# enoche/MMRec

Measured on NVIDIA H100. Metric: graph-prop edges/sec (+ full-catalog scored-items/sec in extra) @ d=64, higher is better.
Workload: dtype f32

## Files before the change

### mmrec_b200/csrc/project_tc.cu

```cuda
#include "tc_common.cuh"

namespace mmrec {

using namespace tc;

constexpr int PJ_M = 128;
constexpr int PJ_KC = 32;
constexpr int PJ_LBO_A = 2064;
constexpr int PJ_A_BYTES = (PJ_KC / 4) * PJ_LBO_A;
constexpr int PJ_CONV = 256;
constexpr int PJ_THREADS = PJ_CONV + 32;
template <int N> constexpr int pj_depth() { return N == 64 ? 3 : (N == 128 ? 2 : 1); }

struct ProjParams {
    const float* table; int64_t F; const int64_t* idx; int64_t n_out;
    const float *Whi, *Wlo;
    int N, n_chunks, chunks_per_split, n_splits, stages, vec_ok, n_tiles;
    float* partial;
    int64_t rows_padded;
};

struct PjSmem {
    uint32_t a0, b0, bars, total, stage_bytes, b_bytes;
};
__host__ __device__ inline PjSmem pj_smem(int N, int stages) {
    PjSmem L;
    L.b_bytes = (uint32_t)N * PJ_KC * 4;
    L.stage_bytes = 2 * PJ_A_BYTES + 2 * L.b_bytes;
    L.a0 = 0;
    L.b0 = 2 * PJ_A_BYTES;
    L.bars = stages * L.stage_bytes;
    L.total = L.bars + 32 * 8;
    return L;
}

template <int N, bool FAST>
__global__ void __launch_bounds__(PJ_THREADS, 1) project_tc_kernel(const ProjParams p) {
    constexpr int PJ_DEPTH = pj_depth<N>();
    extern __shared__ __align__(1024) uint8_t smem[];
    const PjSmem L = pj_smem(N, p.stages);
    const uint32_t sbase = smem_u32(smem);
    const uint32_t bar = sbase + L.bars;
    const int warp = threadIdx.x >> 5, lane = threadIdx.x & 31;
    if (threadIdx.x == 0) {
        for (int s = 0; s < 8; ++s) { mbar_init(bar + s * 8, PJ_CONV); mbar_init(bar + (8 + s) * 8, 1); mbar_init(bar + (16 + s) * 8, PJ_CONV / 32); }
        mbar_fence_init();
    }
    __syncthreads();

    const int tile = blockIdx.x / p.n_splits, sp = blockIdx.x % p.n_splits;
    const int c0 = sp * p.chunks_per_split;
    const int c1 = min(p.n_chunks, c0 + p.chunks_per_split);
    const int n_my = c1 - c0;
    const int rot = n_my > 0 ? ((int)(((int64_t)tile * n_my) / p.n_tiles) / PJ_DEPTH * PJ_DEPTH) % n_my : 0;

    if (warp == PJ_CONV / 32) {
        if (lane == 0) {
            int s = 0;
            uint32_t par = 1;
            for (int c = 0; c < n_my; ++c) {
                mbar_wait(bar + (16 + s) * 8, par);
                mbar_expect_tx(bar + (8 + s) * 8, 2 * L.b_bytes);
                const int64_t off = (int64_t)(c0 + (c + rot) % n_my) * (L.b_bytes / 4);
                bulk_g2s(sbase + s * L.stage_bytes + L.b0, p.Whi + off, L.b_bytes, bar + (8 + s) * 8);
                bulk_g2s(sbase + s * L.stage_bytes + L.b0 + L.b_bytes, p.Wlo + off, L.b_bytes, bar + (8 + s) * 8);
                if (++s == p.stages) { s = 0; par ^= 1; }
            }
        }
        return;
    }
    const int t = threadIdx.x;
    const int g = t >> 7;
    const int kb = t & 7;
    const float* rowp[4];
#pragma unroll
    for (int i = 0; i < 4; ++i) {
        const int64_t r = (int64_t)tile * PJ_M + (t >> 3) + 32 * i;
        rowp[i] = r < p.n_out ? p.table + (p.idx ? p.idx[r] : r) * p.F : nullptr;
    }
    int ld_c = rot;
    const float* kp[4];
#pragma unroll
    for (int i = 0; i < 4; ++i) kp[i] = rowp[i] ? rowp[i] + (int64_t)c0 * PJ_KC + kb * 4 : nullptr;
    auto load_chunk = [&](int c, float4 (&x)[4]) {
        if (FAST) {
            const bool on = c < n_my;
#pragma unroll
            for (int i = 0; i < 4; ++i)
                x[i] = (on && kp[i]) ? __ldg(reinterpret_cast<const float4*>(kp[i] + ld_c * PJ_KC)) : make_float4(0.f, 0.f, 0.f, 0.f);
            if (on && ++ld_c == n_my) ld_c = 0;
            return;
        }
        const int64_t k = (int64_t)(c0 + (c + rot) % n_my) * PJ_KC + kb * 4;
#pragma unroll
        for (int i = 0; i < 4; ++i) {
            float4 v = make_float4(0.f, 0.f, 0.f, 0.f);
            if (rowp[i] && c < n_my) {
                if (p.vec_ok && k + 3 < p.F) v = __ldg(reinterpret_cast<const float4*>(rowp[i] + k));
                else {
                    if (k + 0 < p.F) v.x = __ldg(rowp[i] + k + 0);
                    if (k + 1 < p.F) v.y = __ldg(rowp[i] + k + 1);
                    if (k + 2 < p.F) v.z = __ldg(rowp[i] + k + 2);
                    if (k + 3 < p.F) v.w = __ldg(rowp[i] + k + 3);
                }
            }
            x[i] = v;
        }
    };
    const uint32_t LBO_B = (uint32_t)(N / 8) * 128;
    const uint64_t a_hi0 = smem_desc(sbase + L.a0 + g * 1024, PJ_LBO_A, 128), a_lo0 = smem_desc(sbase + L.a0 + PJ_A_BYTES + g * 1024, PJ_LBO_A, 128);
    const uint64_t b_hi0 = smem_desc(sbase + L.b0, LBO_B, 128), b_lo0 = smem_desc(sbase + L.b0 + L.b_bytes, LBO_B, 128);
    const uint64_t ka = (2 * PJ_LBO_A) >> 4, kbs = (2 * LBO_B) >> 4;
    float acc[N / 2];
#pragma unroll
    for (int i = 0; i < N / 2; ++i) acc[i] = 0.f;
    uint32_t first = 0;
    int prev = 0;
    float4 ringA[PJ_DEPTH][4], ringB[PJ_DEPTH][4];
    int s = 0;
    uint32_t par = 1;
    int done = 0;
    auto fill = [&](int cbase, float4 (&ring)[PJ_DEPTH][4]) {
#pragma unroll
        for (int q = 0; q < PJ_DEPTH; ++q) load_chunk(cbase + q, ring[q]);
    };
    auto drain = [&](int cbase, float4 (&ring)[PJ_DEPTH][4]) {
#pragma unroll
        for (int q = 0; q < PJ_DEPTH; ++q) {
            if (cbase + q < n_my) {
                mbar_wait(bar + (16 + s) * 8, par);
                uint8_t* st = smem + s * L.stage_bytes;
#pragma unroll
                for (int i = 0; i < 4; ++i) {
                    const int r = (t >> 3) + 32 * i;
                    const uint32_t off = kb * PJ_LBO_A + (r >> 3) * 128 + (r & 7) * 16;
                    float4 h, l;
                    split_tf32_trunc(ring[q][i].x, h.x, l.x); split_tf32_trunc(ring[q][i].y, h.y, l.y);
                    split_tf32_trunc(ring[q][i].z, h.z, l.z); split_tf32_trunc(ring[q][i].w, h.w, l.w);
                    *reinterpret_cast<float4*>(st + L.a0 + off) = h;
                    *reinterpret_cast<float4*>(st + L.a0 + PJ_A_BYTES + off) = l;
                }
                fence_proxy_async();
                mbar_arrive(bar + s * 8);
                mbar_wait(bar + s * 8, par ^ 1);
                mbar_wait(bar + (8 + s) * 8, par ^ 1);
                const uint64_t st_off = (uint64_t)(s * L.stage_bytes) >> 4;
                uint64_t a_hi = a_hi0 + st_off, a_lo = a_lo0 + st_off, b_hi = b_hi0 + st_off, b_lo = b_lo0 + st_off;
                wgmma_fence();
#pragma unroll
                for (int j = 0; j < PJ_KC / 8; ++j) {
                    wgmma_tf32<N>(acc, a_hi, b_hi, first);
                    first = 1;
                    wgmma_tf32<N>(acc, a_lo, b_hi, 1);
                    wgmma_tf32<N>(acc, a_hi, b_lo, 1);
                    a_hi += ka; a_lo += ka; b_hi += kbs; b_lo += kbs;
                }
                wgmma_commit();
                if (done++ > 0) {
                    wgmma_wait<1>();
                    warp_arrive(bar + (16 + prev) * 8);
                }
                prev = s;
                if (++s == p.stages) { s = 0; par ^= 1; }
            }
        }
    };
    fill(0, ringA);
    for (int cb = 0; cb < n_my; cb += 2 * PJ_DEPTH) {
        fill(cb + PJ_DEPTH, ringB);
        drain(cb, ringA);
        fill(cb + 2 * PJ_DEPTH, ringA);
        drain(cb + PJ_DEPTH, ringB);
    }
    wgmma_wait<0>();
    wgmma_fence_regs(acc);
    const int w = (t >> 5) & 3;
    const int64_t row0 = (int64_t)tile * PJ_M + g * 64 + w * 16 + (lane >> 2);
#pragma unroll
    for (int h = 0; h < 2; ++h) {
        float* dst = p.partial + ((int64_t)sp * p.rows_padded + row0 + 8 * h) * N + 2 * (lane & 3);
#pragma unroll
        for (int j = 0; j < N / 8; ++j)
            *reinterpret_cast<float2*>(dst + 8 * j) = make_float2(acc[4 * j + 2 * h], acc[4 * j + 2 * h + 1]);
    }
}

__global__ void __launch_bounds__(256) project_reduce_kernel(int64_t n_out, int d, int N, int n_splits, int64_t rows_padded,
                                                             const float* __restrict__ partial, const float* __restrict__ bias,
                                                             int l2, float* __restrict__ Y, int64_t ldy) {
    const int lane = threadIdx.x & 31;
    const int64_t row = (int64_t)blockIdx.x * 8 + (threadIdx.x >> 5);
    if (row >= n_out) return;
    float acc[8];
    float ss = 0.f;
#pragma unroll
    for (int i = 0; i < 8; ++i) {
        const int c = lane + 32 * i;
        float a = 0.f;
        if (c < d) {
            for (int s = 0; s < n_splits; ++s) a += partial[((int64_t)s * rows_padded + row) * N + c];
            if (bias) a += __ldg(bias + c);
            ss += a * a;
        }
        acc[i] = a;
    }
    float inv = 1.f;
    if (l2) { ss = warp_sum(ss); inv = 1.0f / fmaxf(sqrtf(ss), 1e-12f); }
#pragma unroll
    for (int i = 0; i < 8; ++i) {
        const int c = lane + 32 * i;
        if (c < d) Y[row * ldy + c] = l2 ? acc[i] * inv : acc[i];
    }
}

struct PjPlan {
    int N, KP, n_chunks, n_splits, chunks_per_split, stages;
    int64_t n_tiles, rows_padded;
    size_t off_whi, off_wlo, off_partial, total;
};

static bool pj_plan(int64_t n_out, int64_t F, int d, PjPlan& P) {
    if (d > 256 || n_out <= 0 || F < 1) return false;
    P.N = d <= 64 ? 64 : (d <= 128 ? 128 : 256);
    P.KP = (int)((F + PJ_KC - 1) / PJ_KC * PJ_KC);
    P.n_chunks = P.KP / PJ_KC;
    P.n_tiles = (n_out + PJ_M - 1) / PJ_M;
    P.rows_padded = P.n_tiles * PJ_M;
    const int sms = sm_count();
    int splits = (int)(sms / P.n_tiles);
    if (splits < 1) splits = 1;
    if (splits > P.n_chunks / 4) splits = P.n_chunks / 4 > 0 ? P.n_chunks / 4 : 1;
    if (splits > 32) splits = 32;
    P.chunks_per_split = (P.n_chunks + splits - 1) / splits;
    P.n_splits = (P.n_chunks + P.chunks_per_split - 1) / P.chunks_per_split;
    const uint32_t stage = 2 * PJ_A_BYTES + 2 * (uint32_t)P.N * PJ_KC * 4;
    P.stages = (int)((220 * 1024) / stage);
    if (P.stages > 8) P.stages = 8;
    if (P.stages < 2) return false;
    size_t off = 0;
    auto take = [&](size_t bytes) { size_t o = off; off += align_up(bytes, 1024); return o; };
    P.off_whi = take((size_t)P.N * P.KP * 4);
    P.off_wlo = take((size_t)P.N * P.KP * 4);
    P.off_partial = take((size_t)P.n_splits * P.rows_padded * P.N * 4);
    P.total = off + 1024;
    return true;
}

size_t project_tc_workspace_bytes(int64_t n_out, int64_t F, int d) {
    PjPlan P;
    return pj_plan(n_out, F, d, P) ? P.total : 0;
}

template <int R>
static int pack_weights(const float* W, int64_t F, int d, int KP, float* hi, float* lo, cudaStream_t stream) {
    const int64_t total = (int64_t)R * (KP / 4);
    pack_split_kernel<R><<<(unsigned)((total + 255) / 256), 256, 0, stream>>>(d, nullptr, W, F, (int)F, KP, hi, lo, 1);
    MMREC_LAUNCH_CHECK();
    return MMREC_OK;
}

int project_tc(int64_t n_out, const int64_t* idx, const float* table, int64_t F, const float* W, const float* bias, int d,
               int l2_normalize, float* Y, int64_t ldy, void* ws, size_t ws_bytes, cudaStream_t stream) {
    PjPlan P;
    if (!ws || !pj_plan(n_out, F, d, P) || ws_bytes < P.total || F >= (1ll << 31)) return 0;
    char* base = (char*)(((uintptr_t)ws + 1023) & ~(uintptr_t)1023);
    float *Whi = (float*)(base + P.off_whi), *Wlo = (float*)(base + P.off_wlo), *partial = (float*)(base + P.off_partial);
    int rc = P.N == 64 ? pack_weights<64>(W, F, d, P.KP, Whi, Wlo, stream)
                       : (P.N == 128 ? pack_weights<128>(W, F, d, P.KP, Whi, Wlo, stream) : pack_weights<256>(W, F, d, P.KP, Whi, Wlo, stream));
    if (rc) return rc;
    ProjParams p;
    p.table = table; p.F = F; p.idx = idx; p.n_out = n_out; p.Whi = Whi; p.Wlo = Wlo; p.N = P.N; p.n_chunks = P.n_chunks;
    p.chunks_per_split = P.chunks_per_split; p.n_splits = P.n_splits; p.stages = P.stages;
    p.n_tiles = (int)P.n_tiles;
    p.vec_ok = ((F & 3) == 0) && ((((uintptr_t)table) & 15) == 0);
    p.partial = partial; p.rows_padded = P.rows_padded;
    const PjSmem L = pj_smem(P.N, P.stages);
    {
        static bool attr_set[64] = {false};
        int dev = 0;
        MMREC_CUDA(cudaGetDevice(&dev));
        if (dev < 0 || dev >= 64 || !attr_set[dev]) {
            MMREC_CUDA(cudaFuncSetAttribute(project_tc_kernel<64, true>, cudaFuncAttributeMaxDynamicSharedMemorySize, 227 * 1024));
            MMREC_CUDA(cudaFuncSetAttribute(project_tc_kernel<64, false>, cudaFuncAttributeMaxDynamicSharedMemorySize, 227 * 1024));
            MMREC_CUDA(cudaFuncSetAttribute(project_tc_kernel<128, true>, cudaFuncAttributeMaxDynamicSharedMemorySize, 227 * 1024));
            MMREC_CUDA(cudaFuncSetAttribute(project_tc_kernel<128, false>, cudaFuncAttributeMaxDynamicSharedMemorySize, 227 * 1024));
            MMREC_CUDA(cudaFuncSetAttribute(project_tc_kernel<256, true>, cudaFuncAttributeMaxDynamicSharedMemorySize, 227 * 1024));
            MMREC_CUDA(cudaFuncSetAttribute(project_tc_kernel<256, false>, cudaFuncAttributeMaxDynamicSharedMemorySize, 227 * 1024));
            if (dev >= 0 && dev < 64) attr_set[dev] = true;
        }
    }
    const bool fast = p.vec_ok && (F % PJ_KC) == 0;
    const unsigned grid = (unsigned)(P.n_tiles * P.n_splits);
    if (P.N == 64) {
        if (fast) project_tc_kernel<64, true><<<grid, PJ_THREADS, L.total, stream>>>(p);
        else project_tc_kernel<64, false><<<grid, PJ_THREADS, L.total, stream>>>(p);
    } else if (P.N == 128) {
        if (fast) project_tc_kernel<128, true><<<grid, PJ_THREADS, L.total, stream>>>(p);
        else project_tc_kernel<128, false><<<grid, PJ_THREADS, L.total, stream>>>(p);
    } else {
        if (fast) project_tc_kernel<256, true><<<grid, PJ_THREADS, L.total, stream>>>(p);
        else project_tc_kernel<256, false><<<grid, PJ_THREADS, L.total, stream>>>(p);
    }
    MMREC_LAUNCH_CHECK();
    project_reduce_kernel<<<(unsigned)((n_out + 7) / 8), 256, 0, stream>>>(n_out, d, P.N, P.n_splits, P.rows_padded, partial, bias,
                                                                         l2_normalize, Y, ldy);
    MMREC_LAUNCH_CHECK();
    return 1;
}

}
```

Measured before the change: 13.03 billion.

## Stream-K style persistent projection kernel with register reallocation

Replaces the fixed tile×split grid with a persistent grid of at most SM-count CTAs. Each CTA takes a contiguous range of (tile, K-chunk) work units, so work stays balanced when tiles don't divide evenly across SMs. The partial-sum buffer is now indexed by piece within a tile, and the reduce kernel works out how many pieces each tile row has. The producer side grows to a full warpgroup that uses setmaxnreg to hand registers to the consumer warpgroups. Risks include extra reduce passes over partials and dropping the per-tile chunk rotation that previously staggered weight reads.

```diff
diff --git a/mmrec_b200/csrc/project_tc.cu b/mmrec_b200/csrc/project_tc.cu
--- a/mmrec_b200/csrc/project_tc.cu
+++ b/mmrec_b200/csrc/project_tc.cu
@@ -9,13 +9,14 @@
 constexpr int PJ_LBO_A = 2064;
 constexpr int PJ_A_BYTES = (PJ_KC / 4) * PJ_LBO_A;
 constexpr int PJ_CONV = 256;
-constexpr int PJ_THREADS = PJ_CONV + 32;
+constexpr int PJ_THREADS = PJ_CONV + 128;
 template <int N> constexpr int pj_depth() { return N == 64 ? 3 : (N == 128 ? 2 : 1); }
 
 struct ProjParams {
     const float* table; int64_t F; const int64_t* idx; int64_t n_out;
     const float *Whi, *Wlo;
-    int N, n_chunks, chunks_per_split, n_splits, stages, vec_ok, n_tiles;
+    int N, n_chunks, stages, vec_ok;
+    int64_t units;
     float* partial;
     int64_t rows_padded;
 };
@@ -34,6 +35,20 @@
     return L;
 }
 
+__host__ __device__ inline int64_t pj_cta_of(int64_t u, int64_t units, int64_t ctas) { return ((u + 1) * ctas - 1) / units; }
+
+template <class Fn>
+__device__ __forceinline__ void pj_for_each_piece(const ProjParams& p, Fn&& f) {
+    const int64_t u0 = p.units * blockIdx.x / gridDim.x, u1 = p.units * (blockIdx.x + 1) / gridDim.x;
+    for (int64_t u = u0; u < u1;) {
+        const int64_t tile = u / p.n_chunks;
+        const int c0 = (int)(u - tile * p.n_chunks);
+        const int n = u1 - u < p.n_chunks - c0 ? (int)(u1 - u) : p.n_chunks - c0;
+        f(tile, c0, n);
+        u += n;
+    }
+}
+
 template <int N, bool FAST>
 __global__ void __launch_bounds__(PJ_THREADS, 1) project_tc_kernel(const ProjParams p) {
     constexpr int PJ_DEPTH = pj_depth<N>();
@@ -48,65 +63,28 @@
     }
     __syncthreads();
 
-    const int tile = blockIdx.x / p.n_splits, sp = blockIdx.x % p.n_splits;
-    const int c0 = sp * p.chunks_per_split;
-    const int c1 = min(p.n_chunks, c0 + p.chunks_per_split);
-    const int n_my = c1 - c0;
-    const int rot = n_my > 0 ? ((int)(((int64_t)tile * n_my) / p.n_tiles) / PJ_DEPTH * PJ_DEPTH) % n_my : 0;
-
-    if (warp == PJ_CONV / 32) {
-        if (lane == 0) {
+    if (warp >= PJ_CONV / 32) {
+        asm volatile("setmaxnreg.dec.sync.aligned.u32 56;\n" ::: "memory");
+        if (warp == PJ_CONV / 32 && lane == 0) {
             int s = 0;
             uint32_t par = 1;
-            for (int c = 0; c < n_my; ++c) {
-                mbar_wait(bar + (16 + s) * 8, par);
-                mbar_expect_tx(bar + (8 + s) * 8, 2 * L.b_bytes);
-                const int64_t off = (int64_t)(c0 + (c + rot) % n_my) * (L.b_bytes / 4);
-                bulk_g2s(sbase + s * L.stage_bytes + L.b0, p.Whi + off, L.b_bytes, bar + (8 + s) * 8);
-                bulk_g2s(sbase + s * L.stage_bytes + L.b0 + L.b_bytes, p.Wlo + off, L.b_bytes, bar + (8 + s) * 8);
-                if (++s == p.stages) { s = 0; par ^= 1; }
-            }
+            pj_for_each_piece(p, [&](int64_t, int c0, int n_my) {
+                for (int c = 0; c < n_my; ++c) {
+                    mbar_wait(bar + (16 + s) * 8, par);
+                    mbar_expect_tx(bar + (8 + s) * 8, 2 * L.b_bytes);
+                    const int64_t off = (int64_t)(c0 + c) * (L.b_bytes / 4);
+                    bulk_g2s(sbase + s * L.stage_bytes + L.b0, p.Whi + off, L.b_bytes, bar + (8 + s) * 8);
+                    bulk_g2s(sbase + s * L.stage_bytes + L.b0 + L.b_bytes, p.Wlo + off, L.b_bytes, bar + (8 + s) * 8);
+                    if (++s == p.stages) { s = 0; par ^= 1; }
+                }
+            });
         }
         return;
     }
+    asm volatile("setmaxnreg.inc.sync.aligned.u32 224;\n" ::: "memory");
     const int t = threadIdx.x;
     const int g = t >> 7;
     const int kb = t & 7;
-    const float* rowp[4];
-#pragma unroll
-    for (int i = 0; i < 4; ++i) {
-        const int64_t r = (int64_t)tile * PJ_M + (t >> 3) + 32 * i;
-        rowp[i] = r < p.n_out ? p.table + (p.idx ? p.idx[r] : r) * p.F : nullptr;
-    }
-    int ld_c = rot;
-    const float* kp[4];
-#pragma unroll
-    for (int i = 0; i < 4; ++i) kp[i] = rowp[i] ? rowp[i] + (int64_t)c0 * PJ_KC + kb * 4 : nullptr;
-    auto load_chunk = [&](int c, float4 (&x)[4]) {
-        if (FAST) {
-            const bool on = c < n_my;
-#pragma unroll
-            for (int i = 0; i < 4; ++i)
-                x[i] = (on && kp[i]) ? __ldg(reinterpret_cast<const float4*>(kp[i] + ld_c * PJ_KC)) : make_float4(0.f, 0.f, 0.f, 0.f);
-            if (on && ++ld_c == n_my) ld_c = 0;
-            return;
-        }
-        const int64_t k = (int64_t)(c0 + (c + rot) % n_my) * PJ_KC + kb * 4;
-#pragma unroll
-        for (int i = 0; i < 4; ++i) {
-            float4 v = make_float4(0.f, 0.f, 0.f, 0.f);
-            if (rowp[i] && c < n_my) {
-                if (p.vec_ok && k + 3 < p.F) v = __ldg(reinterpret_cast<const float4*>(rowp[i] + k));
-                else {
-                    if (k + 0 < p.F) v.x = __ldg(rowp[i] + k + 0);
-                    if (k + 1 < p.F) v.y = __ldg(rowp[i] + k + 1);
-                    if (k + 2 < p.F) v.z = __ldg(rowp[i] + k + 2);
-                    if (k + 3 < p.F) v.w = __ldg(rowp[i] + k + 3);
-                }
-            }
-            x[i] = v;
-        }
-    };
     const uint32_t LBO_B = (uint32_t)(N / 8) * 128;
     const uint64_t a_hi0 = smem_desc(sbase + L.a0 + g * 1024, PJ_LBO_A, 128), a_lo0 = smem_desc(sbase + L.a0 + PJ_A_BYTES + g * 1024, PJ_LBO_A, 128);
     const uint64_t b_hi0 = smem_desc(sbase + L.b0, LBO_B, 128), b_lo0 = smem_desc(sbase + L.b0 + L.b_bytes, LBO_B, 128);
@@ -114,83 +92,121 @@
     float acc[N / 2];
 #pragma unroll
     for (int i = 0; i < N / 2; ++i) acc[i] = 0.f;
-    uint32_t first = 0;
     int prev = 0;
-    float4 ringA[PJ_DEPTH][4], ringB[PJ_DEPTH][4];
     int s = 0;
     uint32_t par = 1;
     int done = 0;
-    auto fill = [&](int cbase, float4 (&ring)[PJ_DEPTH][4]) {
-#pragma unroll
-        for (int q = 0; q < PJ_DEPTH; ++q) load_chunk(cbase + q, ring[q]);
-    };
-    auto drain = [&](int cbase, float4 (&ring)[PJ_DEPTH][4]) {
-#pragma unroll
-        for (int q = 0; q < PJ_DEPTH; ++q) {
-            if (cbase + q < n_my) {
-                mbar_wait(bar + (16 + s) * 8, par);
-                uint8_t* st = smem + s * L.stage_bytes;
-#pragma unroll
-                for (int i = 0; i < 4; ++i) {
-                    const int r = (t >> 3) + 32 * i;
-                    const uint32_t off = kb * PJ_LBO_A + (r >> 3) * 128 + (r & 7) * 16;
-                    float4 h, l;
-                    split_tf32_trunc(ring[q][i].x, h.x, l.x); split_tf32_trunc(ring[q][i].y, h.y, l.y);
-                    split_tf32_trunc(ring[q][i].z, h.z, l.z); split_tf32_trunc(ring[q][i].w, h.w, l.w);
-                    *reinterpret_cast<float4*>(st + L.a0 + off) = h;
-                    *reinterpret_cast<float4*>(st + L.a0 + PJ_A_BYTES + off) = l;
+    pj_for_each_piece(p, [&](int64_t tile, int c0, int n_my) {
+        const float* rowp[4];
+#pragma unroll
+        for (int i = 0; i < 4; ++i) {
+            const int64_t r = tile * PJ_M + (t >> 3) + 32 * i;
+            rowp[i] = r < p.n_out ? p.table + (p.idx ? p.idx[r] : r) * p.F : nullptr;
+        }
+        const float* kp[4];
+#pragma unroll
+        for (int i = 0; i < 4; ++i) kp[i] = rowp[i] ? rowp[i] + (int64_t)c0 * PJ_KC + kb * 4 : nullptr;
+        auto load_chunk = [&](int c, float4 (&x)[4]) {
+            if (FAST) {
+                const bool on = c < n_my;
+#pragma unroll
+                for (int i = 0; i < 4; ++i)
+                    x[i] = (on && kp[i]) ? __ldg(reinterpret_cast<const float4*>(kp[i] + c * PJ_KC)) : make_float4(0.f, 0.f, 0.f, 0.f);
+                return;
+            }
+            const int64_t k = (int64_t)(c0 + c) * PJ_KC + kb * 4;
+#pragma unroll
+            for (int i = 0; i < 4; ++i) {
+                float4 v = make_float4(0.f, 0.f, 0.f, 0.f);
+                if (rowp[i] && c < n_my) {
+                    if (p.vec_ok && k + 3 < p.F) v = __ldg(reinterpret_cast<const float4*>(rowp[i] + k));
+                    else {
+                        if (k + 0 < p.F) v.x = __ldg(rowp[i] + k + 0);
+                        if (k + 1 < p.F) v.y = __ldg(rowp[i] + k + 1);
+                        if (k + 2 < p.F) v.z = __ldg(rowp[i] + k + 2);
+                        if (k + 3 < p.F) v.w = __ldg(rowp[i] + k + 3);
+                    }
                 }
-                fence_proxy_async();
-                mbar_arrive(bar + s * 8);
-                mbar_wait(bar + s * 8, par ^ 1);
-                mbar_wait(bar + (8 + s) * 8, par ^ 1);
-                const uint64_t st_off = (uint64_t)(s * L.stage_bytes) >> 4;
-                uint64_t a_hi = a_hi0 + st_off, a_lo = a_lo0 + st_off, b_hi = b_hi0 + st_off, b_lo = b_lo0 + st_off;
-                wgmma_fence();
-#pragma unroll
-                for (int j = 0; j < PJ_KC / 8; ++j) {
-                    wgmma_tf32<N>(acc, a_hi, b_hi, first);
-                    first = 1;
-                    wgmma_tf32<N>(acc, a_lo, b_hi, 1);
-                    wgmma_tf32<N>(acc, a_hi, b_lo, 1);
-                    a_hi += ka; a_lo += ka; b_hi += kbs; b_lo += kbs;
+                x[i] = v;
+            }
+        };
+        uint32_t first = 0;
+        float4 ringA[PJ_DEPTH][4], ringB[PJ_DEPTH][4];
+        auto fill = [&](int cbase, float4 (&ring)[PJ_DEPTH][4]) {
+#pragma unroll
+            for (int q = 0; q < PJ_DEPTH; ++q) load_chunk(cbase + q, ring[q]);
+        };
+        auto drain = [&](int cbase, float4 (&ring)[PJ_DEPTH][4]) {
+#pragma unroll
+            for (int q = 0; q < PJ_DEPTH; ++q) {
+                if (cbase + q < n_my) {
+                    mbar_wait(bar + (16 + s) * 8, par);
+                    uint8_t* st = smem + s * L.stage_bytes;
+#pragma unroll
+                    for (int i = 0; i < 4; ++i) {
+                        const int r = (t >> 3) + 32 * i;
+                        const uint32_t off = kb * PJ_LBO_A + (r >> 3) * 128 + (r & 7) * 16;
+                        float4 h, l;
+                        split_tf32_trunc(ring[q][i].x, h.x, l.x); split_tf32_trunc(ring[q][i].y, h.y, l.y);
+                        split_tf32_trunc(ring[q][i].z, h.z, l.z); split_tf32_trunc(ring[q][i].w, h.w, l.w);
+                        *reinterpret_cast<float4*>(st + L.a0 + off) = h;
+                        *reinterpret_cast<float4*>(st + L.a0 + PJ_A_BYTES + off) = l;
+                    }
+                    fence_proxy_async();
+                    mbar_arrive(bar + s * 8);
+                    mbar_wait(bar + s * 8, par ^ 1);
+                    mbar_wait(bar + (8 + s) * 8, par ^ 1);
+                    const uint64_t st_off = (uint64_t)(s * L.stage_bytes) >> 4;
+                    uint64_t a_hi = a_hi0 + st_off, a_lo = a_lo0 + st_off, b_hi = b_hi0 + st_off, b_lo = b_lo0 + st_off;
+                    wgmma_fence();
+#pragma unroll
+                    for (int j = 0; j < PJ_KC / 8; ++j) {
+                        wgmma_tf32<N>(acc, a_hi, b_hi, first);
+                        first = 1;
+                        wgmma_tf32<N>(acc, a_lo, b_hi, 1);
+                        wgmma_tf32<N>(acc, a_hi, b_lo, 1);
+                        a_hi += ka; a_lo += ka; b_hi += kbs; b_lo += kbs;
+                    }
+                    wgmma_commit();
+                    if (done++ > 0) {
+                        wgmma_wait<1>();
+                        warp_arrive(bar + (16 + prev) * 8);
+                    }
+                    prev = s;
+                    if (++s == p.stages) { s = 0; par ^= 1; }
                 }
-                wgmma_commit();
-                if (done++ > 0) {
-                    wgmma_wait<1>();
-                    warp_arrive(bar + (16 + prev) * 8);
-                }
-                prev = s;
-                if (++s == p.stages) { s = 0; par ^= 1; }
             }
-        }
-    };
-    fill(0, ringA);
-    for (int cb = 0; cb < n_my; cb += 2 * PJ_DEPTH) {
-        fill(cb + PJ_DEPTH, ringB);
-        drain(cb, ringA);
-        fill(cb + 2 * PJ_DEPTH, ringA);
-        drain(cb + PJ_DEPTH, ringB);
-    }
-    wgmma_wait<0>();
-    wgmma_fence_regs(acc);
-    const int w = (t >> 5) & 3;
-    const int64_t row0 = (int64_t)tile * PJ_M + g * 64 + w * 16 + (lane >> 2);
-#pragma unroll
-    for (int h = 0; h < 2; ++h) {
-        float* dst = p.partial + ((int64_t)sp * p.rows_padded + row0 + 8 * h) * N + 2 * (lane & 3);
-#pragma unroll
-        for (int j = 0; j < N / 8; ++j)
-            *reinterpret_cast<float2*>(dst + 8 * j) = make_float2(acc[4 * j + 2 * h], acc[4 * j + 2 * h + 1]);
-    }
-}
-
-__global__ void __launch_bounds__(256) project_reduce_kernel(int64_t n_out, int d, int N, int n_splits, int64_t rows_padded,
-                                                             const float* __restrict__ partial, const float* __restrict__ bias,
-                                                             int l2, float* __restrict__ Y, int64_t ldy) {
+        };
+        fill(0, ringA);
+        for (int cb = 0; cb < n_my; cb += 2 * PJ_DEPTH) {
+            fill(cb + PJ_DEPTH, ringB);
+            drain(cb, ringA);
+            fill(cb + 2 * PJ_DEPTH, ringA);
+            drain(cb + PJ_DEPTH, ringB);
+        }
+        wgmma_wait<0>();
+        wgmma_fence_regs(acc);
+        const int64_t piece = blockIdx.x - pj_cta_of(tile * p.n_chunks, p.units, gridDim.x);
+        const int w = (t >> 5) & 3;
+        const int64_t row0 = tile * PJ_M + g * 64 + w * 16 + (lane >> 2);
+#pragma unroll
+        for (int h = 0; h < 2; ++h) {
+            float* dst = p.partial + (piece * p.rows_padded + row0 + 8 * h) * N + 2 * (lane & 3);
+#pragma unroll
+            for (int j = 0; j < N / 8; ++j)
+                *reinterpret_cast<float2*>(dst + 8 * j) = make_float2(acc[4 * j + 2 * h], acc[4 * j + 2 * h + 1]);
+        }
+    });
+}
+
+__global__ void __launch_bounds__(256) project_reduce_kernel(int64_t n_out, int d, int N, int n_chunks, int64_t units, int ctas,
+                                                             int64_t rows_padded, const float* __restrict__ partial,
+                                                             const float* __restrict__ bias, int l2, float* __restrict__ Y, int64_t ldy) {
     const int lane = threadIdx.x & 31;
     const int64_t row = (int64_t)blockIdx.x * 8 + (threadIdx.x >> 5);
     if (row >= n_out) return;
+    const int64_t u = row / PJ_M * n_chunks;
+    const int n_pieces = (int)(pj_cta_of(u + n_chunks - 1, units, ctas) - pj_cta_of(u, units, ctas)) + 1;
     float acc[8];
     float ss = 0.f;
 #pragma unroll
@@ -198,7 +214,7 @@
         const int c = lane + 32 * i;
         float a = 0.f;
         if (c < d) {
-            for (int s = 0; s < n_splits; ++s) a += partial[((int64_t)s * rows_padded + row) * N + c];
+            for (int s = 0; s < n_pieces; ++s) a += partial[((int64_t)s * rows_padded + row) * N + c];
             if (bias) a += __ldg(bias + c);
             ss += a * a;
         }
@@ -214,8 +230,8 @@
 }
 
 struct PjPlan {
-    int N, KP, n_chunks, n_splits, chunks_per_split, stages;
-    int64_t n_tiles, rows_padded;
+    int N, KP, n_chunks, ctas, max_pieces, stages;
+    int64_t n_tiles, rows_padded, units;
     size_t off_whi, off_wlo, off_partial, total;
 };
 
@@ -226,13 +242,11 @@
     P.n_chunks = P.KP / PJ_KC;
     P.n_tiles = (n_out + PJ_M - 1) / PJ_M;
     P.rows_padded = P.n_tiles * PJ_M;
-    const int sms = sm_count();
-    int splits = (int)(sms / P.n_tiles);
-    if (splits < 1) splits = 1;
-    if (splits > P.n_chunks / 4) splits = P.n_chunks / 4 > 0 ? P.n_chunks / 4 : 1;
-    if (splits > 32) splits = 32;
-    P.chunks_per_split = (P.n_chunks + splits - 1) / splits;
-    P.n_splits = (P.n_chunks + P.chunks_per_split - 1) / P.chunks_per_split;
+    P.units = P.n_tiles * P.n_chunks;
+    P.ctas = (int)std::max<int64_t>(1, std::min<int64_t>(sm_count(), P.units / 4));
+    P.max_pieces = 1;
+    for (int64_t u = 0; u < P.units; u += P.n_chunks)
+        P.max_pieces = (int)std::max<int64_t>(P.max_pieces, pj_cta_of(u + P.n_chunks - 1, P.units, P.ctas) - pj_cta_of(u, P.units, P.ctas) + 1);
     const uint32_t stage = 2 * PJ_A_BYTES + 2 * (uint32_t)P.N * PJ_KC * 4;
     P.stages = (int)((220 * 1024) / stage);
     if (P.stages > 8) P.stages = 8;
@@ -241,7 +255,7 @@
     auto take = [&](size_t bytes) { size_t o = off; off += align_up(bytes, 1024); return o; };
     P.off_whi = take((size_t)P.N * P.KP * 4);
     P.off_wlo = take((size_t)P.N * P.KP * 4);
-    P.off_partial = take((size_t)P.n_splits * P.rows_padded * P.N * 4);
+    P.off_partial = take((size_t)P.max_pieces * P.rows_padded * P.N * 4);
     P.total = off + 1024;
     return true;
 }
@@ -270,8 +284,7 @@
     if (rc) return rc;
     ProjParams p;
     p.table = table; p.F = F; p.idx = idx; p.n_out = n_out; p.Whi = Whi; p.Wlo = Wlo; p.N = P.N; p.n_chunks = P.n_chunks;
-    p.chunks_per_split = P.chunks_per_split; p.n_splits = P.n_splits; p.stages = P.stages;
-    p.n_tiles = (int)P.n_tiles;
+    p.stages = P.stages; p.units = P.units;
     p.vec_ok = ((F & 3) == 0) && ((((uintptr_t)table) & 15) == 0);
     p.partial = partial; p.rows_padded = P.rows_padded;
     const PjSmem L = pj_smem(P.N, P.stages);
@@ -290,7 +303,7 @@
         }
     }
     const bool fast = p.vec_ok && (F % PJ_KC) == 0;
-    const unsigned grid = (unsigned)(P.n_tiles * P.n_splits);
+    const unsigned grid = (unsigned)P.ctas;
     if (P.N == 64) {
         if (fast) project_tc_kernel<64, true><<<grid, PJ_THREADS, L.total, stream>>>(p);
         else project_tc_kernel<64, false><<<grid, PJ_THREADS, L.total, stream>>>(p);
@@ -302,8 +315,8 @@
         else project_tc_kernel<256, false><<<grid, PJ_THREADS, L.total, stream>>>(p);
     }
     MMREC_LAUNCH_CHECK();
-    project_reduce_kernel<<<(unsigned)((n_out + 7) / 8), 256, 0, stream>>>(n_out, d, P.N, P.n_splits, P.rows_padded, partial, bias,
-                                                                         l2_normalize, Y, ldy);
+    project_reduce_kernel<<<(unsigned)((n_out + 7) / 8), 256, 0, stream>>>(n_out, d, P.N, P.n_chunks, P.units, P.ctas, P.rows_padded,
+                                                                         partial, bias, l2_normalize, Y, ldy);
     MMREC_LAUNCH_CHECK();
     return 1;
 }
```

After: 13.03 billion, median of 6. Within noise of the previous version (+0.0%).
